# floatingtrees/video-VAE

Hardware: AMD Instinct MI355X
Metric: video frames/sec (fwd+bwd) at Bx3x16x256x256 (higher is better)
Workload: dtype bf16; 1 GPU; C3: full VideoVAE (enc 9 / dec 12 FactoredAttention + 3D-conv UNet) train step, B=4/GPU x 3x16x256x256, bf16 compute, fp32 params, recon+KL loss, clip+Adam; flavour=model, params=170631304, global_batch=4, frames_per_clip=16, parallelism=dp1, launch_mode=hipgraph(fwd+bwd) + eager all-reduce/clip/Adam

## Files before the change

video_vae_amd/csrc/attn_rows.hpp:

```cpp
#pragma once
#include "common.hpp"

namespace {

template <typename T_> struct Vw;
template <> struct Vw<float> { static constexpr int n = 4; };
template <> struct Vw<bf16_t> { static constexpr int n = 8; };

template <typename T_, int D, int LPR> struct Slice {
    static constexpr int DL = D / LPR;
    static constexpr int HL = DL / 2;
    static constexpr int H = D / 2;
    static constexpr int V = Vw<T_>::n < HL ? Vw<T_>::n : HL;
    static_assert(HL % V == 0 && HL >= 4, "slice halves must be whole vectors");
    static __device__ __forceinline__ int ch(int r, int p) { return r < HL ? p * HL + r : H + p * HL + (r - HL); }
    static __device__ __forceinline__ int lo(int p) { return p * HL; }
    static __device__ __forceinline__ int hi(int p) { return H + p * HL; }
};

__device__ __forceinline__ float dpp_xor1(float v) {
    return __int_as_float(__builtin_amdgcn_mov_dpp(__float_as_int(v), 0xB1, 0xf, 0xf, true));
}
__device__ __forceinline__ float dpp_xor2(float v) {
    return __int_as_float(__builtin_amdgcn_mov_dpp(__float_as_int(v), 0x4E, 0xf, 0xf, true));
}
template <int LPR> __device__ __forceinline__ float lpr_sum(float v) {
    static_assert(LPR == 1 || LPR == 2 || LPR == 4, "frames are split over at most a lane quad");
    if (LPR >= 2) v += dpp_xor1(v);
    if (LPR >= 4) v += dpp_xor2(v);
    return v;
}
template <int LPR> __device__ __forceinline__ float frames_sum(float v) { return butterfly_sum<32, LPR>(v); }

template <typename T_, int D, int LPR>
__device__ __forceinline__ void load_row(const T_* __restrict__ row, int p, float (&r)[D / LPR]) {
    using S = Slice<T_, D, LPR>;
#pragma unroll
    for (int half = 0; half < 2; ++half) {
        const T_* src = row + (half ? S::hi(p) : S::lo(p));
#pragma unroll
        for (int c = 0; c < S::HL / S::V; ++c) {
            float t[S::V];
            VecIO<T_, S::V>::load(src + c * S::V, t);
#pragma unroll
            for (int e = 0; e < S::V; ++e) r[half * S::HL + c * S::V + e] = t[e];
        }
    }
}
template <typename T_, int D, int LPR>
__device__ __forceinline__ void store_row(T_* __restrict__ row, int p, const float (&r)[D / LPR]) {
    using S = Slice<T_, D, LPR>;
#pragma unroll
    for (int half = 0; half < 2; ++half) {
        T_* dst = row + (half ? S::hi(p) : S::lo(p));
#pragma unroll
        for (int c = 0; c < S::HL / S::V; ++c) {
            float t[S::V];
#pragma unroll
            for (int e = 0; e < S::V; ++e) t[e] = r[half * S::HL + c * S::V + e];
            VecIO<T_, S::V>::store(dst + c * S::V, t);
        }
    }
}
template <typename T_, int D, int LPR>
__device__ __forceinline__ void load_tab(const float* __restrict__ row, int p, float (&r)[D / LPR]) {
    using S = Slice<T_, D, LPR>;
#pragma unroll
    for (int i = 0; i < S::DL; ++i) r[i] = row[S::ch(i, p)];
}

template <int DL, int LPR, int D>
__device__ __forceinline__ float xhat_row(float (&x)[DL], float eps) {
    float s = 0.f, ss = 0.f;
#pragma unroll
    for (int i = 0; i < DL; ++i) { s += x[i]; ss += x[i] * x[i]; }
    s = lpr_sum<LPR>(s); ss = lpr_sum<LPR>(ss);
    const float mean = s / D;
    float var = ss / D - mean * mean;
    var = var < 0.f ? 0.f : var;
    const float rstd = rsqrtf(var + eps);
#pragma unroll
    for (int i = 0; i < DL; ++i) x[i] = (x[i] - mean) * rstd;
    return rstd;
}

template <typename T_, int D, int LPR>
__device__ __forceinline__ void ln_rope_row(float (&x)[D / LPR], int p, const float* __restrict__ scale, float eps,
                                            const float* __restrict__ cosr, const float* __restrict__ sinr) {
    using S = Slice<T_, D, LPR>;
    xhat_row<S::DL, LPR, D>(x, eps);
#pragma unroll
    for (int i = 0; i < S::HL; ++i) {
        const int cl = S::ch(i, p), chh = S::ch(i + S::HL, p);
        float lo = x[i] * scale[cl], hi = x[i + S::HL] * scale[chh];
        round2<T_>(lo, hi);
        float a = lo * cosr[cl], b = -hi * sinr[cl], c = hi * cosr[chh], e = lo * sinr[chh];
        round2<T_>(a, b);
        round2<T_>(c, e);
        float y0 = a + b, y1 = c + e;
        round2<T_>(y0, y1);
        x[i] = y0; x[i + S::HL] = y1;
    }
}

template <typename T_, int D, int LPR>
__device__ __forceinline__ void rope_ln_bwd_row(float (&g)[D / LPR], float (&xh)[D / LPR], int p, float rstd,
                                                const float* __restrict__ scale, const float* __restrict__ cosr,
                                                const float* __restrict__ sinr) {
    using S = Slice<T_, D, LPR>;
#pragma unroll
    for (int i = 0; i < S::HL; ++i) {
        const float lo = g[i], hi = g[i + S::HL];
        const int cl = S::ch(i, p), chh = S::ch(i + S::HL, p);
        g[i] = lo * cosr[cl] + hi * sinr[chh];
        g[i + S::HL] = hi * cosr[chh] - lo * sinr[cl];
    }
    float sc[S::DL];
    load_tab<T_, D, LPR>(scale, p, sc);
    float s1 = 0.f, s2 = 0.f;
#pragma unroll
    for (int i = 0; i < S::DL; ++i) {
        const float dxh = g[i] * sc[i];
        s1 += dxh; s2 += dxh * xh[i];
    }
    s1 = lpr_sum<LPR>(s1) / D; s2 = lpr_sum<LPR>(s2) / D;
#pragma unroll
    for (int i = 0; i < S::DL; ++i) {
        const float dy = g[i], x = xh[i];
        g[i] = rstd * (dy * sc[i] - s1 - x * s2);
        xh[i] = dy * x;
    }
}

template <typename T_, int D, int LPR>
__device__ __forceinline__ void ln_rope_row_reg(float (&x)[D / LPR], float eps, const float (&sc)[D / LPR], const float (&cs)[D / LPR],
                                                const float (&sn)[D / LPR]) {
    using S = Slice<T_, D, LPR>;
    xhat_row<S::DL, LPR, D>(x, eps);
#pragma unroll
    for (int i = 0; i < S::HL; ++i) {
        float lo = x[i] * sc[i], hi = x[i + S::HL] * sc[i + S::HL];
        round2<T_>(lo, hi);
        float a = lo * cs[i], b = -hi * sn[i], c = hi * cs[i + S::HL], e = lo * sn[i + S::HL];
        round2<T_>(a, b);
        round2<T_>(c, e);
        float y0 = a + b, y1 = c + e;
        round2<T_>(y0, y1);
        x[i] = y0; x[i + S::HL] = y1;
    }
}
template <typename T_, int D, int LPR>
__device__ __forceinline__ void rope_ln_bwd_row_reg(float (&g)[D / LPR], float (&xh)[D / LPR], float rstd, const float (&sc)[D / LPR],
                                                    const float (&cs)[D / LPR], const float (&sn)[D / LPR]) {
    using S = Slice<T_, D, LPR>;
#pragma unroll
    for (int i = 0; i < S::HL; ++i) {
        const float lo = g[i], hi = g[i + S::HL];
        g[i] = lo * cs[i] + hi * sn[i + S::HL];
        g[i + S::HL] = hi * cs[i + S::HL] - lo * sn[i];
    }
    float s1 = 0.f, s2 = 0.f;
#pragma unroll
    for (int i = 0; i < S::DL; ++i) {
        const float dxh = g[i] * sc[i];
        s1 += dxh; s2 += dxh * xh[i];
    }
    s1 = lpr_sum<LPR>(s1) / D; s2 = lpr_sum<LPR>(s2) / D;
#pragma unroll
    for (int i = 0; i < S::DL; ++i) {
        const float dy = g[i], x = xh[i];
        g[i] = rstd * (dy * sc[i] - s1 - x * s2);
        xh[i] = dy * x;
    }
}

}
```

video_vae_amd/csrc/attn_spatial.hip:

```cpp
#include "attn_tile32.hpp"

#ifndef SATTN_PROBE
#define SATTN_PROBE 0
#endif

namespace {

struct SAttnDims { int A, S, H; float eps; };

template <int NT, int S_>
struct RawRows {
    static constexpr int RPP = NT / 4;
    static constexpr int PASSES = (S_ + RPP - 1) / RPP;
    uint4 v[PASSES][2];
    __device__ __forceinline__ void fetch(const bf16_t* __restrict__ src, long tok0, int ld) {
        const int p = threadIdx.x & 3;
#pragma unroll
        for (int i = 0; i < PASSES; ++i) {
            const int row = (threadIdx.x >> 2) + i * RPP;
            if (S_ % RPP == 0 || row < S_) {
                const bf16_t* r = src + (tok0 + row) * ld;
                v[i][0] = *reinterpret_cast<const uint4*>(r + 8 * p);
                v[i][1] = *reinterpret_cast<const uint4*>(r + 32 + 8 * p);
            } else {
                v[i][0] = make_uint4(0u, 0u, 0u, 0u);
                v[i][1] = make_uint4(0u, 0u, 0u, 0u);
            }
        }
    }
    static __device__ __forceinline__ void unpack(const uint4 (&u)[2], float (&x)[16]) {
        const uint32_t w[8] = {u[0].x, u[0].y, u[0].z, u[0].w, u[1].x, u[1].y, u[1].z, u[1].w};
#pragma unroll
        for (int i = 0; i < 8; ++i) { x[2 * i] = __uint_as_float(w[i] << 16); x[2 * i + 1] = __uint_as_float(w[i] & 0xffff0000u); }
    }
    __device__ __forceinline__ void put_raw(unsigned char* img) const {
        const int p = threadIdx.x & 3;
#pragma unroll
        for (int i = 0; i < PASSES; ++i) {
            const int row = (threadIdx.x >> 2) + i * RPP;
            if (S_ % RPP == 0 || row < S_) {
                *reinterpret_cast<uint4*>(img + img_off(row, p)) = v[i][0];
                *reinterpret_cast<uint4*>(img + img_off(row, 4 + p)) = v[i][1];
            }
        }
    }
    template <class Tabs>
    __device__ __forceinline__ void put_norm(unsigned char* img, const float (&sc)[16], float eps, const Tabs& t) const {
        const int p = threadIdx.x & 3;
#pragma unroll
        for (int i = 0; i < PASSES; ++i) {
            const int row = (threadIdx.x >> 2) + i * RPP;
            if (S_ % RPP == 0 || row < S_) {
                float x[16];
                unpack(v[i], x);
                ln_rope_row_reg<bf16_t, SD, 4>(x, eps, sc, t.cs[i], t.sn[i]);
                float lo[8], hi[8];
#pragma unroll
                for (int e = 0; e < 8; ++e) { lo[e] = x[e]; hi[e] = x[8 + e]; }
                VecIO<bf16_t, 8>::store(reinterpret_cast<bf16_t*>(img + img_off(row, p)), lo);
                VecIO<bf16_t, 8>::store(reinterpret_cast<bf16_t*>(img + img_off(row, 4 + p)), hi);
            }
        }
    }
};
template <int NT, int S_>
struct RowTabs {
    static constexpr int RPP = NT / 4, PASSES = (S_ + RPP - 1) / RPP;
    float cs[PASSES][16], sn[PASSES][16];
    __device__ __forceinline__ void fetch(const float* __restrict__ cosT, const float* __restrict__ sinT) {
        const int p = threadIdx.x & 3;
#pragma unroll
        for (int i = 0; i < PASSES; ++i) {
            int row = (threadIdx.x >> 2) + i * RPP;
            if (S_ % RPP != 0 && row >= S_) row = 0;
            load_tab<bf16_t, SD, 4>(cosT + (long)row * SD, p, cs[i]);
            load_tab<bf16_t, SD, 4>(sinT + (long)row * SD, p, sn[i]);
        }
    }
};

template <int NKB>
__global__ __launch_bounds__(256, 2) void sattn_fwd_kernel(const bf16_t* __restrict__ qkv, int ld, bf16_t* __restrict__ out, int ldo,
                                                           float* __restrict__ lse2, const float* __restrict__ q_scale,
                                                           const float* __restrict__ k_scale, const float* __restrict__ cosT,
                                                           const float* __restrict__ sinT, SAttnDims d)
{
    extern __shared__ __attribute__((aligned(16))) unsigned char smem[];
    constexpr int S = 32 * NKB;
    unsigned char* Ks = smem;
    unsigned char* Vs = smem + S * SROW;
    const int lane = threadIdx.x & 63, wave = threadIdx.x >> 6;
    unsigned char* scr = smem + 2 * S * SROW + wave * SCR_BYTES;
    const int a = blockIdx.x / d.H, h = blockIdx.x - a * d.H;
    const int HD = d.H * SD;
    const long tok0 = (long)a * S;
    const bf16_t* base = qkv + h * SD;

    if (!(SATTN_PROBE & 1)) {
        RawRows<256, S> rk, rv;
        RowTabs<256, S> tabs;
        float sck[16];
        rk.fetch(base + HD, tok0, ld);
        tabs.fetch(cosT, sinT);
        load_tab<bf16_t, SD, 4>(k_scale, threadIdx.x & 3, sck);
        rv.fetch(base + 2 * HD, tok0, ld);
        rk.put_norm(Ks, sck, d.eps, tabs);
        rv.put_raw(Vs);
    }
    __syncthreads();

    const int j = lane & 31, kh = lane >> 5;
    const FragAddr fa(lane);
    const float c2 = rsqrtf((float)SD) * 1.44269504088896341f;

    for (int qb = wave; qb < NKB && !(SATTN_PROBE & 2); qb += 4) {
        const int qrow = qb * 32 + j;
        bf16x8 qf[4];
        {
            float x[2][16], cs[2][16], sn[2][16], sc[16];
#pragma unroll
            for (int hf = 0; hf < 2; ++hf) {
                const long rr = qb * 32 + 16 * hf + (lane >> 2);
                load_row<bf16_t, SD, 4>(base + (tok0 + rr) * ld, lane & 3, x[hf]);
                load_tab<bf16_t, SD, 4>(cosT + rr * SD, lane & 3, cs[hf]);
                load_tab<bf16_t, SD, 4>(sinT + rr * SD, lane & 3, sn[hf]);
            }
            load_tab<bf16_t, SD, 4>(q_scale, lane & 3, sc);
#pragma unroll
            for (int hf = 0; hf < 2; ++hf) {
                ln_rope_row_reg<bf16_t, SD, 4>(x[hf], d.eps, sc, cs[hf], sn[hf]);
                wave_lds_fence();
                rows_put(scr, lane, x[hf]);
                wave_lds_fence();
                if ((j >> 4) == hf) {
#pragma unroll
                    for (int ks = 0; ks < 4; ++ks)
                        qf[ks] = *reinterpret_cast<const bf16x8*>(scr + (j & 15) * SROW + (((2 * ks + kh) ^ gsw(j & 15)) << 4));
                }
            }
        }

        constexpr int G = NKB < 4 ? NKB : 4;
        float m = -3.0e38f, l = 0.f;
// ... 2 lines not shown
        for (int dt = 0; dt < 2; ++dt)
#pragma unroll
            for (int e = 0; e < 16; ++e) o[dt][e] = 0.f;
#pragma unroll 1
        for (int kb0 = 0; kb0 < NKB; kb0 += G) {
            f32x16 s[G];
            float mg = m;
#pragma unroll
            for (int g = 0; g < G; ++g) {
                if (kb0 + g < NKB) {
#pragma unroll
                    for (int e = 0; e < 16; ++e) s[g][e] = 0.f;
#pragma unroll
                    for (int ks = 0; ks < 4; ++ks) {
                        s[g] = __builtin_amdgcn_mfma_f32_32x32x16_bf16(fa.rowfrag(Ks, kb0 + g, ks), qf[ks], s[g], 0, 0, 0);
                    }
#pragma unroll
                    for (int e = 0; e < 16; ++e) mg = fmaxf(mg, s[g][e]);
                }
            }
            mg = fmaxf(mg, xor32(mg));
            if (kb0 > 0) {
                const float alpha = exp2_fast((m - mg) * c2);
                l *= alpha;
#pragma unroll
                for (int dt = 0; dt < 2; ++dt)
#pragma unroll
                    for (int e = 0; e < 16; ++e) o[dt][e] *= alpha;
            }
            m = mg;
            const float mc2 = m * c2;
#pragma unroll
            for (int g = 0; g < G; ++g) {
                if (kb0 + g < NKB) {
#pragma unroll
                    for (int u = 0; u < 2; ++u) {
                        float pv[8];
#pragma unroll
                        for (int e = 0; e < 8; ++e) { pv[e] = exp2_fast(__builtin_fmaf(s[g][8 * u + e], c2, -mc2)); l += pv[e]; }
                        const bf16x8 pf = pack8(pv);
#pragma unroll
                        for (int dt = 0; dt < 2; ++dt)
                            o[dt] = __builtin_amdgcn_mfma_f32_32x32x16_bf16(fa.trfrag(Vs, kb0 + g, u, dt), pf, o[dt], 0, 0, 0);
                    }
                }
            }
        }
        l += xor32(l);
        const float inv = 1.f / l;
        float og[2][16];
#pragma unroll
        for (int dt = 0; dt < 2; ++dt)
#pragma unroll
            for (int e = 0; e < 16; ++e) og[dt][e] = o[dt][e] * inv;
#pragma unroll
        for (int hf = 0; hf < 2; ++hf) {
            wave_lds_fence();
            acc_half_put(scr, j, kh, hf, og);
            wave_lds_fence();
            float x[16];
            rows_get(scr, lane, x);
            store_row<bf16_t, SD, 4>(out + (tok0 + qb * 32 + 16 * hf + (lane >> 2)) * ldo + h * SD, lane & 3, x);
        }
        if (kh == 0) lse2[((long)a * d.H + h) * S + qrow] = m * c2 + log2f(l);
    }
}

template <int NKB>
__global__ __launch_bounds__(512) void sattn_bwd_kernel(const bf16_t* __restrict__ qkv, int ld, const bf16_t* __restrict__ out, int ldo,
                                                           const bf16_t* __restrict__ dout, int lddo, const float* __restrict__ lse2,
                                                           bf16_t* __restrict__ dqkv, int lddq, const float* __restrict__ q_scale,
                                                           const float* __restrict__ k_scale, const float* __restrict__ cosT,
                                                           const float* __restrict__ sinT, float* __restrict__ part, SAttnDims d)
{
    extern __shared__ __attribute__((aligned(16))) unsigned char smem[];
    constexpr int S = 32 * NKB;
    unsigned char* Qs = smem;
    unsigned char* Ks = smem + S * SROW;
    unsigned char* Vs = smem + 2 * S * SROW;
    unsigned char* Gs = smem + 3 * S * SROW;
    float* lseS = reinterpret_cast<float*>(smem + 4 * S * SROW);
    float* delS = lseS + S;
    float* red = delS + S;
    const int lane = threadIdx.x & 63, wave = threadIdx.x >> 6;
    unsigned char* scr = reinterpret_cast<unsigned char*>(red + 16 * SD) + wave * SCR_BYTES;
    const int a = blockIdx.x / d.H, h = blockIdx.x - a * d.H;
    const int HD = d.H * SD;
    const long tok0 = (long)a * S;
    const bf16_t* base = qkv + h * SD;
    const bf16_t* gbase = dout + h * SD;
    const int j = lane & 31, kh = lane >> 5;
    const FragAddr fa(lane);
    const float sm_scale = rsqrtf((float)SD);
    const float c2 = sm_scale * 1.44269504088896341f;

    if (!(SATTN_PROBE & 1)) {
        typedef RawRows<512, S> RR;
        RR rv, rg, ro, rq, rk;
        RowTabs<512, S> tabs;
        float scq[16], sck[16];
        rq.fetch(base, tok0, ld);
        rk.fetch(base + HD, tok0, ld);
        tabs.fetch(cosT, sinT);
        load_tab<bf16_t, SD, 4>(q_scale, threadIdx.x & 3, scq);
        load_tab<bf16_t, SD, 4>(k_scale, threadIdx.x & 3, sck);
        rv.fetch(base + 2 * HD, tok0, ld);
        rg.fetch(gbase, tok0, lddo);
        ro.fetch(out + h * SD, tok0, ldo);
        float lse_r[RR::PASSES];
#pragma unroll
        for (int i = 0; i < RR::PASSES; ++i) {
            const int row = (threadIdx.x >> 2) + i * RR::RPP;
            lse_r[i] = row < S ? lse2[((long)a * d.H + h) * S + row] : 0.f;
        }
        rq.put_norm(Qs, scq, d.eps, tabs);
        rk.put_norm(Ks, sck, d.eps, tabs);
        rv.put_raw(Vs);
        rg.put_raw(Gs);
#pragma unroll
        for (int i = 0; i < RR::PASSES; ++i) {
            const int row = (threadIdx.x >> 2) + i * RR::RPP;
            float go[16], oo[16];
            RR::unpack(rg.v[i], go);
            RR::unpack(ro.v[i], oo);
            float dl = 0.f;
#pragma unroll
            for (int e = 0; e < 16; ++e) dl += go[e] * oo[e];
            dl = lpr_sum<4>(dl);
            if ((threadIdx.x & 3) == 0 && row < S) { delS[row] = dl; lseS[row] = lse_r[i]; }
        }
    }
    auto put_v_tile = [&](const float (&g)[2][16], int row0) {
#pragma unroll
        for (int hf = 0; hf < 2; ++hf) {
            wave_lds_fence();
            acc_half_put(scr, j, kh, hf, g);
            wave_lds_fence();
            float x[16];
            rows_get(scr, lane, x);
            store_row<bf16_t, SD, 4>(dqkv + (tok0 + row0 + 16 * hf + (lane >> 2)) * lddq + 2 * HD + h * SD, lane & 3, x);
        }
    };
    struct RowCtx { float xr[2][16], cs[2][16], sn[2][16], sc[16]; };
    auto qk_loads = [&](RowCtx& c, int row0, int which, const float* __restrict__ scale) {
        const int p = lane & 3;
#pragma unroll
        for (int hf = 0; hf < 2; ++hf) {
            const long rr = row0 + 16 * hf + (lane >> 2);
            load_row<bf16_t, SD, 4>(base + which * HD + (tok0 + rr) * ld, p, c.xr[hf]);
            load_tab<bf16_t, SD, 4>(cosT + rr * SD, p, c.cs[hf]);
            load_tab<bf16_t, SD, 4>(sinT + rr * SD, p, c.sn[hf]);
        }
        load_tab<bf16_t, SD, 4>(scale, p, c.sc);
    };
    auto qk_finish = [&](RowCtx& c, const float (&g)[2][16], int row0, int which) {
        const int p = lane & 3;
        float ds[16];
#pragma unroll
        for (int hf = 0; hf < 2; ++hf) {
            const int rr = row0 + 16 * hf + (lane >> 2);
            wave_lds_fence();
            acc_half_put(scr, j, kh, hf, g);
            wave_lds_fence();
            float gx[16];
            rows_get(scr, lane, gx);
            const float rstd = xhat_row<16, 4, SD>(c.xr[hf], d.eps);
            rope_ln_bwd_row_reg<bf16_t, SD, 4>(gx, c.xr[hf], rstd, c.sc, c.cs[hf], c.sn[hf]);
            store_row<bf16_t, SD, 4>(dqkv + (tok0 + rr) * lddq + which * HD + h * SD, p, gx);
#pragma unroll
            for (int i = 0; i < 16; ++i) ds[i] = hf ? ds[i] + c.xr[hf][i] : c.xr[hf][i];
        }
#pragma unroll
        for (int i = 0; i < 16; ++i) {
            const float t = frames_sum<4>(ds[i]);
            if (lane < 4) red[(wave * 2 + which) * SD + Slice<bf16_t, SD, 4>::ch(i, p)] = t;
        }
    };
    static_assert(NKB <= 8, "one key tile and one query tile per wave: the red[] slots are written once");
    for (int i = threadIdx.x; i < 16 * SD; i += 512) red[i] = 0.f;
    __syncthreads();

    for (int kt = wave; kt < NKB && !(SATTN_PROBE & 2); kt += 8) {
        bf16x8 kc[4], vc[4];
#pragma unroll
        for (int ks = 0; ks < 4; ++ks) { kc[ks] = fa.rowfrag(Ks, kt, ks); vc[ks] = fa.rowfrag(Vs, kt, ks); }
        f32x16 dv[2], dk[2];
#pragma unroll
        for (int dt = 0; dt < 2; ++dt)
#pragma unroll
            for (int e = 0; e < 16; ++e) { dv[dt][e] = 0.f; dk[dt][e] = 0.f; }
        bf16x8 qr[4], gr[4];
#pragma unroll
        for (int ks = 0; ks < 4; ++ks) { qr[ks] = fa.rowfrag(Qs, 0, ks); gr[ks] = fa.rowfrag(Gs, 0, ks); }
#pragma unroll 1
        for (int qb = 0; qb < NKB; ++qb) {
            f32x16 s, dp;
#pragma unroll
            for (int e = 0; e < 16; ++e) { s[e] = 0.f; dp[e] = 0.f; }
#pragma unroll
            for (int ks = 0; ks < 4; ++ks) {
                s = __builtin_amdgcn_mfma_f32_32x32x16_bf16(qr[ks], kc[ks], s, 0, 0, 0);
                dp = __builtin_amdgcn_mfma_f32_32x32x16_bf16(gr[ks], vc[ks], dp, 0, 0, 0);
            }
            bf16x8 gt[2][2], qt[2][2];
            float4 l4[4], d4[4];
#pragma unroll
            for (int u = 0; u < 2; ++u)
#pragma unroll
                for (int dt = 0; dt < 2; ++dt) { gt[u][dt] = fa.trfrag(Gs, qb, u, dt); qt[u][dt] = fa.trfrag(Qs, qb, u, dt); }
#pragma unroll
            for (int i = 0; i < 4; ++i) {
                l4[i] = *reinterpret_cast<const float4*>(lseS + qb * 32 + 8 * i + 4 * kh);
                d4[i] = *reinterpret_cast<const float4*>(delS + qb * 32 + 8 * i + 4 * kh);
            }
            {
                const int nb = qb + 1 < NKB ? qb + 1 : qb;
#pragma unroll
                for (int ks = 0; ks < 4; ++ks) { qr[ks] = fa.rowfrag(Qs, nb, ks); gr[ks] = fa.rowfrag(Gs, nb, ks); }
            }
#pragma unroll
            for (int u = 0; u < 2; ++u) {
                float p8[8], s8[8];
#pragma unroll
                for (int hh = 0; hh < 2; ++hh) {
                    const float4 lv = l4[2 * u + hh], dv4 = d4[2 * u + hh];
                    const float lq[4] = {lv.x, lv.y, lv.z, lv.w}, dq4[4] = {dv4.x, dv4.y, dv4.z, dv4.w};
#pragma unroll
                    for (int e = 0; e < 4; ++e) {
                        const float pe = exp2_fast(s[8 * u + 4 * hh + e] * c2 - lq[e]);
                        p8[4 * hh + e] = pe;
                        s8[4 * hh + e] = pe * (dp[8 * u + 4 * hh + e] - dq4[e]);
                    }
                }
                const bf16x8 pf = pack8(p8), sf = pack8(s8);
#pragma unroll
                for (int dt = 0; dt < 2; ++dt) {
                    dv[dt] = __builtin_amdgcn_mfma_f32_32x32x16_bf16(gt[u][dt], pf, dv[dt], 0, 0, 0);
                    dk[dt] = __builtin_amdgcn_mfma_f32_32x32x16_bf16(qt[u][dt], sf, dk[dt], 0, 0, 0);
                }
            }
        }
        RowCtx c;
        qk_loads(c, kt * 32, 1, k_scale);
        float g[2][16];
#pragma unroll
        for (int dt = 0; dt < 2; ++dt)
#pragma unroll
            for (int r = 0; r < 16; ++r) g[dt][r] = dv[dt][r];
        put_v_tile(g, kt * 32);
#pragma unroll
        for (int dt = 0; dt < 2; ++dt)
#pragma unroll
            for (int r = 0; r < 16; ++r) g[dt][r] = dk[dt][r] * sm_scale;
        qk_finish(c, g, kt * 32, 1);
    }

    for (int qt = wave; qt < NKB && !(SATTN_PROBE & 4); qt += 8) {
        const int qrow = qt * 32 + j;
        bf16x8 qc[4], gc[4];
#pragma unroll
        for (int ks = 0; ks < 4; ++ks) { qc[ks] = fa.rowfrag(Qs, qt, ks); gc[ks] = fa.rowfrag(Gs, qt, ks); }
        const float lq = lseS[qrow], dl = delS[qrow];
        f32x16 dq[2];
#pragma unroll
        for (int dt = 0; dt < 2; ++dt)
#pragma unroll
            for (int e = 0; e < 16; ++e) dq[dt][e] = 0.f;
        bf16x8 kr[4], vr[4];
#pragma unroll
        for (int ks = 0; ks < 4; ++ks) { kr[ks] = fa.rowfrag(Ks, 0, ks); vr[ks] = fa.rowfrag(Vs, 0, ks); }
#pragma unroll 1
        for (int kb = 0; kb < NKB; ++kb) {
            f32x16 s, dp;
#pragma unroll
            for (int e = 0; e < 16; ++e) { s[e] = 0.f; dp[e] = 0.f; }
#pragma unroll
            for (int ks = 0; ks < 4; ++ks) {
                s = __builtin_amdgcn_mfma_f32_32x32x16_bf16(kr[ks], qc[ks], s, 0, 0, 0);
                dp = __builtin_amdgcn_mfma_f32_32x32x16_bf16(vr[ks], gc[ks], dp, 0, 0, 0);
            }
            bf16x8 kt2[2][2];
#pragma unroll
            for (int u = 0; u < 2; ++u)
#pragma unroll
                for (int dt = 0; dt < 2; ++dt) kt2[u][dt] = fa.trfrag(Ks, kb, u, dt);
            {
                const int nb = kb + 1 < NKB ? kb + 1 : kb;
#pragma unroll
                for (int ks = 0; ks < 4; ++ks) { kr[ks] = fa.rowfrag(Ks, nb, ks); vr[ks] = fa.rowfrag(Vs, nb, ks); }
            }
#pragma unroll
            for (int u = 0; u < 2; ++u) {
                float s8[8];
#pragma unroll
                for (int e = 0; e < 8; ++e) s8[e] = exp2_fast(s[8 * u + e] * c2 - lq) * (dp[8 * u + e] - dl);
                const bf16x8 sf = pack8(s8);
#pragma unroll
                for (int dt = 0; dt < 2; ++dt)
                    dq[dt] = __builtin_amdgcn_mfma_f32_32x32x16_bf16(kt2[u][dt], sf, dq[dt], 0, 0, 0);
            }
        }
        float g[2][16];
#pragma unroll
        for (int dt = 0; dt < 2; ++dt)
#pragma unroll
            for (int r = 0; r < 16; ++r) g[dt][r] = dq[dt][r] * sm_scale;
        RowCtx c;
        qk_loads(c, qt * 32, 0, q_scale);
        qk_finish(c, g, qt * 32, 0);
    }

    __syncthreads();
    if (threadIdx.x < 2 * SD) {
        const int t = threadIdx.x;
        float tot = 0.f;
#pragma unroll
        for (int w = 0; w < 8; ++w) tot += red[w * 2 * SD + t];
        part[(long)blockIdx.x * 2 * SD + t] = tot;
    }
}

bool sattn_ok(int S, int D, int dtype) { return D == SD && dtype == VVAE_DT_BF16 && S >= 32 && S <= 256 && S % 32 == 0; }

template <int NKB>
int launch_sattn_bwd(const void* qkv, int ld, const void* out, int ldo, const void* dout, int lddo, const float* lse2, void* dqkv, int lddq,
                     const float* qs, const float* ks, const float* cosT, const float* sinT, float* part, SAttnDims d, hipStream_t s)
{
    constexpr int lds = 4 * 32 * NKB * SROW + 2 * 32 * NKB * 4 + 16 * SD * 4 + 8 * SCR_BYTES;
    auto k = sattn_bwd_kernel<NKB>;
    static bool attr_done = false;
    if (!attr_done && lds > 48 * 1024) {
        hipError_t e = hipFuncSetAttribute((const void*)k, hipFuncAttributeMaxDynamicSharedMemorySize, lds);
        if (e != hipSuccess) return (int)e;
        attr_done = true;
    }
    hipLaunchKernelGGL(k, dim3(d.A * d.H), dim3(512), lds, s, (const bf16_t*)qkv, ld, (const bf16_t*)out, ldo, (const bf16_t*)dout, lddo, lse2,
                       (bf16_t*)dqkv, lddq, qs, ks, cosT, sinT, part, d);
    VVAE_LAUNCH_CHECK();
    return 0;
}

template <int NKB>
int launch_sattn_fwd(const void* qkv, int ld, void* out, int ldo, float* lse2, const float* qs, const float* ks, const float* cosT,
                     const float* sinT, SAttnDims d, hipStream_t s)
{
    constexpr int lds = 2 * 32 * NKB * SROW + 4 * SCR_BYTES;
    auto k = sattn_fwd_kernel<NKB>;
    static bool attr_done = false;
    if (!attr_done && lds > 48 * 1024) {
        hipError_t e = hipFuncSetAttribute((const void*)k, hipFuncAttributeMaxDynamicSharedMemorySize, lds);
        if (e != hipSuccess) return (int)e;
        attr_done = true;
    }
    hipLaunchKernelGGL(k, dim3(d.A * d.H), dim3(256), lds, s, (const bf16_t*)qkv, ld, (bf16_t*)out, ldo, lse2, qs, ks, cosT, sinT, d);
    VVAE_LAUNCH_CHECK();
    return 0;
}

}

#define SATTN_DISPATCH(FN, ...)                                                         \
    switch (S / 32) {                                                                   \
        case 1: return FN<1>(__VA_ARGS__); case 2: return FN<2>(__VA_ARGS__);           \
        case 3: return FN<3>(__VA_ARGS__); case 4: return FN<4>(__VA_ARGS__);           \
        case 5: return FN<5>(__VA_ARGS__); case 6: return FN<6>(__VA_ARGS__);           \
        case 7: return FN<7>(__VA_ARGS__); default: return FN<8>(__VA_ARGS__);          \
    }

extern "C" int vvae_spatial_attn_supported(int S, int D, int dtype) { return sattn_ok(S, D, dtype) ? 1 : 0; }

extern "C" int vvae_spatial_attn_fwd(const void* qkv, int ld, void* out, int ldo, float* lse2, const float* q_scale, const float* k_scale,
                                     const float* cos_table, const float* sin_table, int A, int S, int heads, int D, float eps, int dtype,
                                     void* stream)
{
    if (!qkv || !out || !lse2 || !q_scale || !k_scale || !cos_table || !sin_table || A <= 0 || heads <= 0 || !sattn_ok(S, D, dtype) ||
        ld < 3 * heads * D || ldo < heads * D || ld % 8 || ldo % 8 || ((uintptr_t)qkv % 16) || ((uintptr_t)out % 16))
        return VVAE_ERR_BAD_ARG;
    SAttnDims d{A, S, heads, eps};
    hipStream_t s = (hipStream_t)stream;
    SATTN_DISPATCH(launch_sattn_fwd, qkv, ld, out, ldo, lse2, q_scale, k_scale, cos_table, sin_table, d, s);
}

extern "C" int vvae_spatial_attn_bwd(const void* qkv, int ld, const void* out, int ldo, const void* dout, int lddo, const float* lse2,
                                     void* dqkv, int lddq, const float* q_scale, const float* k_scale, const float* cos_table,
                                     const float* sin_table, float* part, int A, int S, int heads, int D, float eps, int dtype, void* stream)
{
    if (!qkv || !out || !dout || !lse2 || !dqkv || !part || !q_scale || !k_scale || !cos_table || !sin_table || A <= 0 || heads <= 0 ||
        !sattn_ok(S, D, dtype) || ld < 3 * heads * D || lddq < 3 * heads * D || ldo < heads * D || lddo < heads * D || ld % 8 || ldo % 8 ||
        lddo % 8 || lddq % 8 || ((uintptr_t)qkv % 16) || ((uintptr_t)out % 16) || ((uintptr_t)dout % 16) || ((uintptr_t)dqkv % 16))
        return VVAE_ERR_BAD_ARG;
    SAttnDims d{A, S, heads, eps};
    hipStream_t s = (hipStream_t)stream;
    SATTN_DISPATCH(launch_sattn_bwd, qkv, ld, out, ldo, dout, lddo, lse2, dqkv, lddq, q_scale, k_scale, cos_table, sin_table, part, d, s);
}
```

video_vae_amd/csrc/attn_temporal_mfma.hip:

```cpp
#include "common.hpp"

namespace tmfma {

typedef __bf16 bf16x8 __attribute__((ext_vector_type(8)));
typedef short s16x4v __attribute__((ext_vector_type(4)));

constexpr int T = 16, D = 64;
constexpr int PITCH = 160;
constexpr int IMG = T * PITCH;

struct Dims { int A, heads, mask_div, inner; float eps; long items; };

__device__ __forceinline__ long token_of(const Dims& d, int a, int row) {
    return (long)(a / d.inner) * T * d.inner + (long)row * d.inner + (a % d.inner);
}

__device__ __forceinline__ void unpack8(const uint4& r, float* v) {
    const uint32_t w[4] = {r.x, r.y, r.z, r.w};
#pragma unroll
    for (int i = 0; i < 4; ++i) { v[2 * i] = __uint_as_float(w[i] << 16); v[2 * i + 1] = __uint_as_float(w[i] & 0xffff0000u); }
}
__device__ __forceinline__ uint4 pack8(const float* v) {
    uint32_t w[4];
#pragma unroll
    for (int i = 0; i < 4; ++i) w[i] = (uint32_t)f2bf(v[2 * i]) | ((uint32_t)f2bf(v[2 * i + 1]) << 16);
    return make_uint4(w[0], w[1], w[2], w[3]);
}
__device__ __forceinline__ bf16x8 frag8(const uint4& r) { return __builtin_bit_cast(bf16x8, r); }
__device__ __forceinline__ s16x4v pack4(float a, float b, float c, float e) {
    s16x4v r = {(short)f2bf(a), (short)f2bf(b), (short)f2bf(c), (short)f2bf(e)};
    return r;
}
__device__ __forceinline__ s16x4v tr4(const unsigned char* p) {
    typedef __attribute__((address_space(3))) s16x4v* lds_ptr;
    return __builtin_amdgcn_ds_read_tr16_b64_v4i16((lds_ptr)p);
}
__device__ __forceinline__ f32x4 mfma32(const bf16x8& a, const bf16x8& b, f32x4 c) { return __builtin_amdgcn_mfma_f32_16x16x32_bf16(a, b, c, 0, 0, 0); }
__device__ __forceinline__ f32x4 mfma16(const s16x4v& a, const s16x4v& b, f32x4 c) { return __builtin_amdgcn_mfma_f32_16x16x16bf16_1k(a, b, c, 0, 0, 0); }

__device__ __forceinline__ float psum(float v) { return butterfly_sum<32, 16>(v); }
__device__ __forceinline__ float pmax(float v) { v = fmaxf(v, xor_lane<32>(v)); return fmaxf(v, xor_lane<16>(v)); }

__device__ __forceinline__ float xhat16(float (&x)[16], float eps) {
    float s = 0.f, ss = 0.f;
#pragma unroll
    for (int i = 0; i < 16; ++i) { s += x[i]; ss += x[i] * x[i]; }
    s = psum(s); ss = psum(ss);
    const float mean = s * (1.f / D);
    float var = ss * (1.f / D) - mean * mean;
    var = var < 0.f ? 0.f : var;
    const float rstd = rsqrtf(var + eps);
#pragma unroll
    for (int i = 0; i < 16; ++i) x[i] = (x[i] - mean) * rstd;
    return rstd;
}
__device__ __forceinline__ void ln_rope16(float (&x)[16], const float* __restrict__ sc, float eps, const float* __restrict__ cs,
                                          const float* __restrict__ sn) {
    xhat16(x, eps);
#pragma unroll
    for (int i = 0; i < 8; ++i) {
        float lo = x[i] * sc[i], hi = x[i + 8] * sc[i + 8];
        round2<bf16_t>(lo, hi);
        float a = lo * cs[i], b = -hi * sn[i], c = hi * cs[i + 8], e = lo * sn[i + 8];
        round2<bf16_t>(a, b);
        round2<bf16_t>(c, e);
        float y0 = a + b, y1 = c + e;
        round2<bf16_t>(y0, y1);
        x[i] = y0; x[i + 8] = y1;
    }
}
__device__ __forceinline__ void tab16(const float* __restrict__ row, int p, float (&r)[16]) {
    const float4* lo = reinterpret_cast<const float4*>(row + 8 * p);
    const float4* hi = reinterpret_cast<const float4*>(row + 32 + 8 * p);
    const float4 a = lo[0], b = lo[1], c = hi[0], e = hi[1];
    r[0] = a.x; r[1] = a.y; r[2] = a.z; r[3] = a.w; r[4] = b.x; r[5] = b.y; r[6] = b.z; r[7] = b.w;
    r[8] = c.x; r[9] = c.y; r[10] = c.z; r[11] = c.w; r[12] = e.x; r[13] = e.y; r[14] = e.z; r[15] = e.w;
}
__device__ __forceinline__ void norm_row(const bf16_t* __restrict__ g, int p, const float (&sc)[16], float eps, const float (&cs)[16],
                                         const float (&sn)[16], uint4& f0, uint4& f1) {
    float x[16];
    unpack8(*reinterpret_cast<const uint4*>(g + 8 * p), x);
    unpack8(*reinterpret_cast<const uint4*>(g + 32 + 8 * p), x + 8);
    ln_rope16(x, sc, eps, cs, sn);
    f0 = pack8(x); f1 = pack8(x + 8);
}
__device__ __forceinline__ void put_row(unsigned char* img, int t, int p, const uint4& f0, const uint4& f1) {
    *reinterpret_cast<uint4*>(img + t * PITCH + 16 * p) = f0;
    *reinterpret_cast<uint4*>(img + t * PITCH + 64 + 16 * p) = f1;
}
__device__ __forceinline__ void wave_lds_fence() {
    __builtin_amdgcn_wave_barrier();
    __builtin_amdgcn_s_waitcnt(0xc07f);
    __builtin_amdgcn_wave_barrier();
}
__device__ __forceinline__ s16x4v tr_rows(const unsigned char* img, int p, int i, int tile) {
    return tr4(img + (4 * p + (i >> 2)) * PITCH + 32 * tile + 8 * (i & 3));
}

__global__ __launch_bounds__(256) void tattn16_fwd_mfma(const bf16_t* __restrict__ qkv, int ld, bf16_t* __restrict__ out, int ldo,
                                                       float* __restrict__ lse, const float* __restrict__ q_scale,
                                                       const float* __restrict__ k_scale, const float* __restrict__ cosT,
                                                       const float* __restrict__ sinT, const uint8_t* __restrict__ mask, Dims d)
{
    __shared__ __attribute__((aligned(16))) unsigned char smem[4 * IMG];
    const int lane = threadIdx.x & 63, wave = threadIdx.x >> 6;
    const int t = lane & 15, p = lane >> 4;
    const long item = (long)blockIdx.x * 4 + wave;
    if (item >= d.items) return;
    const int a = (int)(item / d.heads), h = (int)(item % d.heads);
    const int HD = d.heads * D;
    const long tok = token_of(d, a, t);
    const bf16_t* g = qkv + tok * ld + h * D;
    unsigned char* vimg = smem + wave * IMG;

// ... 317 lines not shown
```

video_vae_amd/csrc/attn_tile32.hpp:

```cpp
#pragma once
#include "attn_rows.hpp"

namespace {

typedef __bf16 bf16x8 __attribute__((ext_vector_type(8)));
typedef short s16x4v __attribute__((ext_vector_type(4)));

constexpr int SD = 64;
constexpr int SROW = SD * 2;

__device__ __forceinline__ int gsw(int row) { return (((row >> 1) & 1) << 2) | (((row >> 3) & 1) << 1) | ((row >> 2) & 1); }

__device__ __forceinline__ float xor32(float v) { return xor_lane<32>(v); }

__device__ __forceinline__ bf16x8 pack8(const float (&v)[8])
{
    s16x8 r;
#pragma unroll
    for (int e = 0; e < 8; ++e) r[e] = (short)f2bf(v[e]);
    return __builtin_bit_cast(bf16x8, r);
}

__device__ __forceinline__ bf16x8 tr_pair(const unsigned char* p0, const unsigned char* p1)
{
    typedef __attribute__((address_space(3))) s16x4v* lds_ptr;
    const s16x4v lo = __builtin_amdgcn_ds_read_tr16_b64_v4i16((lds_ptr)p0);
    const s16x4v hi = __builtin_amdgcn_ds_read_tr16_b64_v4i16((lds_ptr)p1);
    s16x8 v = {lo[0], lo[1], lo[2], lo[3], hi[0], hi[1], hi[2], hi[3]};
    return __builtin_bit_cast(bf16x8, v);
}

__device__ __forceinline__ int img_off(int row, int c) { return row * SROW + ((c ^ gsw(row)) << 4); }
struct FragAddr {
    int row[4], tr[2][2];
    __device__ __forceinline__ FragAddr(int lane) {
        const int j = lane & 31, kh = lane >> 5, p4 = lane & 3, qr = (lane >> 2) & 3, mh = (lane >> 4) & 1;
        const int gj = gsw(j), gl = (((qr >> 1) & 1) << 2) | kh;
#pragma unroll
        for (int ks = 0; ks < 4; ++ks) row[ks] = j * SROW + (((2 * ks + kh) ^ gj) << 4);
#pragma unroll
        for (int dt = 0; dt < 2; ++dt)
#pragma unroll
            for (int x = 0; x < 2; ++x)
                tr[dt][x] = (4 * kh + qr + 8 * x) * SROW + (((2 * (2 * dt + mh) + (p4 >> 1)) ^ (gl | (x << 1))) << 4) + (p4 & 1) * 8;
    }
    __device__ __forceinline__ bf16x8 rowfrag(const unsigned char* img, int blk, int ks) const {
        return *reinterpret_cast<const bf16x8*>(img + blk * 32 * SROW + row[ks]);
    }
    __device__ __forceinline__ bf16x8 trfrag(const unsigned char* img, int blk, int u, int dt) const {
        const unsigned char* b = img + (blk * 32 + 16 * u) * SROW;
        return tr_pair(b + tr[dt][0], b + tr[dt][1]);
    }
};

constexpr int SCR_BYTES = 16 * SROW;

__device__ __forceinline__ void wave_lds_fence()
{
    __builtin_amdgcn_wave_barrier();
    __builtin_amdgcn_s_waitcnt(0xc07f);
    __builtin_amdgcn_wave_barrier();
}

__device__ __forceinline__ void acc_half_put(unsigned char* scr, int j, int kh, int hf, const float (&g)[2][16])
{
    if ((j >> 4) == hf) {
        const int row = j & 15, gs = gsw(row);
        unsigned char* r = scr + row * SROW + kh * 8;
#pragma unroll
        for (int dt = 0; dt < 2; ++dt)
#pragma unroll
            for (int rg = 0; rg < 4; ++rg) {
                uint2 o;
                o.x = (uint32_t)f2bf(g[dt][4 * rg]) | ((uint32_t)f2bf(g[dt][4 * rg + 1]) << 16);
                o.y = (uint32_t)f2bf(g[dt][4 * rg + 2]) | ((uint32_t)f2bf(g[dt][4 * rg + 3]) << 16);
                *reinterpret_cast<uint2*>(r + (((4 * dt + rg) ^ gs) << 4)) = o;
            }
    }
}
__device__ __forceinline__ void rows_put(unsigned char* scr, int lane, const float (&x)[16])
{
    const int row = lane >> 2, p = lane & 3;
    float lo[8], hi[8];
#pragma unroll
    for (int e = 0; e < 8; ++e) { lo[e] = x[e]; hi[e] = x[8 + e]; }
    VecIO<bf16_t, 8>::store(reinterpret_cast<bf16_t*>(scr + img_off(row, p)), lo);
    VecIO<bf16_t, 8>::store(reinterpret_cast<bf16_t*>(scr + img_off(row, 4 + p)), hi);
}
__device__ __forceinline__ void rows_get(const unsigned char* scr, int lane, float (&x)[16])
{
    const int row = lane >> 2, p = lane & 3;
    float lo[8], hi[8];
    VecIO<bf16_t, 8>::load(reinterpret_cast<const bf16_t*>(scr + img_off(row, p)), lo);
    VecIO<bf16_t, 8>::load(reinterpret_cast<const bf16_t*>(scr + img_off(row, 4 + p)), hi);
#pragma unroll
    for (int e = 0; e < 8; ++e) { x[e] = lo[e]; x[8 + e] = hi[e]; }
}

__device__ __forceinline__ float exp2_fast(float x) { return __builtin_amdgcn_exp2f(x); }

}
```

video_vae_amd/csrc/common.hpp:

```cpp
#pragma once
#include <hip/hip_runtime.h>
#include <stdint.h>

#define VVAE_DT_F32 0
#define VVAE_DT_BF16 1

#define VVAE_ERR_BAD_ARG 1001
#define VVAE_ERR_WORKSPACE 1002
#define VVAE_ERR_LIBRARY 1003

typedef uint16_t bf16_t;

typedef float f32x4 __attribute__((ext_vector_type(4)));
typedef float f32x16 __attribute__((ext_vector_type(16)));
typedef short s16x8 __attribute__((ext_vector_type(8)));
typedef short s16x4 __attribute__((ext_vector_type(4)));

__device__ __forceinline__ float bf2f(bf16_t b) { return __uint_as_float(((uint32_t)b) << 16); }

__device__ __forceinline__ bf16_t f2bf(float f) {
    __bf16 h = (__bf16)f;
    return __builtin_bit_cast(bf16_t, h);
}

__device__ __forceinline__ float ldf(const float* p) { return *p; }
__device__ __forceinline__ float ldf(const bf16_t* p) { return bf2f(*p); }
__device__ __forceinline__ void stf(float* p, float v) { *p = v; }
__device__ __forceinline__ void stf(bf16_t* p, float v) { *p = f2bf(v); }

template <typename T> __device__ __forceinline__ float round_to(float v);
template <> __device__ __forceinline__ float round_to<float>(float v) { return v; }
template <> __device__ __forceinline__ float round_to<bf16_t>(float v) { return bf2f(f2bf(v)); }
template <typename T> __device__ __forceinline__ void round2(float& a, float& b);
template <> __device__ __forceinline__ void round2<float>(float&, float&) {}
template <> __device__ __forceinline__ void round2<bf16_t>(float& a, float& b) {
    typedef __bf16 bf16x2_t __attribute__((ext_vector_type(2)));
    typedef float f32x2_t __attribute__((ext_vector_type(2)));
    const f32x2_t v = {a, b};
    const uint32_t w = __builtin_bit_cast(uint32_t, __builtin_convertvector(v, bf16x2_t));
    a = __uint_as_float(w << 16);
    b = __uint_as_float(w & 0xffff0000u);
}

__device__ __forceinline__ void vvae_phase_barrier()
{
    __builtin_amdgcn_sched_barrier(0);
    __builtin_amdgcn_s_barrier();
    __builtin_amdgcn_sched_barrier(0);
}

template <typename T, int VEC> struct VecIO;

template <> struct VecIO<float, 4> {
    static __device__ __forceinline__ void load(const float* p, float (&v)[4]) {
        float4 t = *reinterpret_cast<const float4*>(p);
        v[0] = t.x; v[1] = t.y; v[2] = t.z; v[3] = t.w;
    }
    static __device__ __forceinline__ void store(float* p, const float (&v)[4]) {
        *reinterpret_cast<float4*>(p) = make_float4(v[0], v[1], v[2], v[3]);
    }
};
template <> struct VecIO<float, 1> {
    static __device__ __forceinline__ void load(const float* p, float (&v)[1]) { v[0] = *p; }
    static __device__ __forceinline__ void store(float* p, const float (&v)[1]) { *p = v[0]; }
};
template <> struct VecIO<bf16_t, 8> {
    static __device__ __forceinline__ void load(const bf16_t* p, float (&v)[8]) {
        uint4 t = *reinterpret_cast<const uint4*>(p);
        uint32_t w[4] = {t.x, t.y, t.z, t.w};
#pragma unroll
        for (int i = 0; i < 4; ++i) {
            v[2 * i] = __uint_as_float(w[i] << 16);
            v[2 * i + 1] = __uint_as_float(w[i] & 0xffff0000u);
        }
    }
    static __device__ __forceinline__ void store(bf16_t* p, const float (&v)[8]) {
        uint32_t w[4];
#pragma unroll
        for (int i = 0; i < 4; ++i) w[i] = (uint32_t)f2bf(v[2 * i]) | ((uint32_t)f2bf(v[2 * i + 1]) << 16);
        *reinterpret_cast<uint4*>(p) = make_uint4(w[0], w[1], w[2], w[3]);
    }
};
template <> struct VecIO<bf16_t, 4> {
    static __device__ __forceinline__ void load(const bf16_t* p, float (&v)[4]) {
        uint2 t = *reinterpret_cast<const uint2*>(p);
        v[0] = __uint_as_float(t.x << 16); v[1] = __uint_as_float(t.x & 0xffff0000u);
        v[2] = __uint_as_float(t.y << 16); v[3] = __uint_as_float(t.y & 0xffff0000u);
    }
    static __device__ __forceinline__ void store(bf16_t* p, const float (&v)[4]) {
        uint2 t;
        t.x = (uint32_t)f2bf(v[0]) | ((uint32_t)f2bf(v[1]) << 16);
        t.y = (uint32_t)f2bf(v[2]) | ((uint32_t)f2bf(v[3]) << 16);
        *reinterpret_cast<uint2*>(p) = t;
    }
};
template <> struct VecIO<bf16_t, 1> {
    static __device__ __forceinline__ void load(const bf16_t* p, float (&v)[1]) { v[0] = bf2f(*p); }
    static __device__ __forceinline__ void store(bf16_t* p, const float (&v)[1]) { *p = f2bf(v[0]); }
};

template <typename T> struct VecWidth;
template <> struct VecWidth<float> { static constexpr int value = 4; };
template <> struct VecWidth<bf16_t> { static constexpr int value = 8; };

template <int CTRL> __device__ __forceinline__ unsigned dpp_u32(unsigned v) {
    return (unsigned)__builtin_amdgcn_update_dpp(0, (int)v, CTRL, 0xf, 0xf, true);
}
template <int O> __device__ __forceinline__ unsigned xor_lane_u32(unsigned v) {
    static_assert(O == 1 || O == 2 || O == 4 || O == 8 || O == 16 || O == 32, "one address bit at a time");
    if constexpr (O == 1) return dpp_u32<0xB1>(v);
    else if constexpr (O == 2) return dpp_u32<0x4E>(v);
    else if constexpr (O == 4) return dpp_u32<0x1B>(dpp_u32<0x141>(v));
    else if constexpr (O == 8) return dpp_u32<0x128>(v);
    else if constexpr (O == 16) {
        const auto r = __builtin_amdgcn_permlane16_swap(v, v, false, false);
        return (threadIdx.x & 16) ? r[0] : r[1];
    } else {
        const auto r = __builtin_amdgcn_permlane32_swap(v, v, false, false);
        return (threadIdx.x & 32) ? r[0] : r[1];
    }
}
template <int O> __device__ __forceinline__ float xor_lane(float v) { return __uint_as_float(xor_lane_u32<O>(__float_as_uint(v))); }
template <int O> __device__ __forceinline__ double xor_lane(double v) {
    const unsigned long long u = __builtin_bit_cast(unsigned long long, v);
    const unsigned lo = xor_lane_u32<O>((unsigned)u), hi = xor_lane_u32<O>((unsigned)(u >> 32));
    return __builtin_bit_cast(double, ((unsigned long long)hi << 32) | lo);
}
template <int HI, int LO, typename F> __device__ __forceinline__ F butterfly_sum(F v) {
    static_assert(HI >= LO && LO >= 1, "bit range");
    v += xor_lane<HI>(v);
    if constexpr (HI > LO) return butterfly_sum<HI / 2, LO>(v);
    else return v;
}

__device__ __forceinline__ float wave_sum(float v) { return butterfly_sum<32, 1>(v); }
__device__ __forceinline__ double wave_sum(double v) { return butterfly_sum<32, 1>(v); }

__device__ __forceinline__ float sigmoidf_(float x) { return __builtin_amdgcn_rcpf(1.0f + __expf(-x)); }

static inline int ceil_div(long a, long b) { return (int)((a + b - 1) / b); }

__global__ static void vvae_zero_words_kernel(uint32_t* __restrict__ p, long n)
{
    for (long i = (long)blockIdx.x * blockDim.x + threadIdx.x; i < n; i += (long)gridDim.x * blockDim.x) p[i] = 0u;
}
static inline hipError_t vvae_zero_async(void* p, size_t bytes, hipStream_t s)
{
    const long n = (long)(bytes / 4);
    if (n <= 0) return hipSuccess;
    long blocks = (n + 255) / 256;
    if (blocks > 1024) blocks = 1024;
    hipLaunchKernelGGL(vvae_zero_words_kernel, dim3((unsigned)blocks), dim3(256), 0, s, (uint32_t*)p, n);
    return hipGetLastError();
}
__global__ static void vvae_reduce_rows_kernel(const float* __restrict__ part, int rows, long stride, int ncols, float* __restrict__ out0, int n0,
                                               float* __restrict__ out1)
{
    __shared__ float red[8][32];
    const int cl = threadIdx.x & 31, rl = threadIdx.x >> 5;
    const int c = blockIdx.x * 32 + cl;
    float s = 0.f;
    if (c < ncols) {
        for (int r0 = rl; r0 < rows; r0 += 8 * 8) {
            float v[8];
#pragma unroll
            for (int i = 0; i < 8; ++i) {
                const int r = r0 + 8 * i;
                v[i] = r < rows ? part[(long)r * stride + c] : 0.f;
            }
#pragma unroll
            for (int i = 0; i < 8; ++i) s += v[i];
        }
    }
    red[rl][cl] = s;
    __syncthreads();
    if (rl == 0 && c < ncols) {
        const float t = ((red[0][cl] + red[1][cl]) + (red[2][cl] + red[3][cl])) + ((red[4][cl] + red[5][cl]) + (red[6][cl] + red[7][cl]));
        if (c < n0) out0[c] = t;
        else if (out1) out1[c - n0] = t;
    }
}

#define VVAE_LAUNCH_CHECK() do { hipError_t e_ = hipGetLastError(); if (e_ != hipSuccess) return (int)e_; } while (0)
```

Before: 1913 frames/s.

## Cache LayerNorm row stats in LDS for spatial attention backward and pack bf16 pairwise

The spatial attention backward kernel now writes each Q/K row's mean and rstd to LDS during the forward-normalise pass and reuses them in the gradient pass, instead of recomputing the row reduction with lane shuffles. Scalar bf16 conversions are replaced with a paired float-to-bf16x2 vector conversion in several pack helpers. Butterfly sums for offsets 16/32 now add both outputs of permlane swap directly, avoiding a lane-dependent select. The kernel uses more LDS, which may reduce occupancy.

```diff
diff --git a/video_vae_amd/csrc/attn_rows.hpp b/video_vae_amd/csrc/attn_rows.hpp
--- a/video_vae_amd/csrc/attn_rows.hpp
+++ b/video_vae_amd/csrc/attn_rows.hpp
@@ -47,6 +47,13 @@
         }
     }
 }
+template <typename T_, int V> struct RowIO : VecIO<T_, V> {};
+template <> struct RowIO<bf16_t, 8> : VecIO<bf16_t, 8> {
+    static __device__ __forceinline__ void store(bf16_t* p, const float (&v)[8]) {
+        *reinterpret_cast<uint4*>(p) = make_uint4(pack2bf(v[0], v[1]), pack2bf(v[2], v[3]), pack2bf(v[4], v[5]), pack2bf(v[6], v[7]));
+    }
+};
+
 template <typename T_, int D, int LPR>
 __device__ __forceinline__ void store_row(T_* __restrict__ row, int p, const float (&r)[D / LPR]) {
     using S = Slice<T_, D, LPR>;
@@ -58,7 +65,7 @@
             float t[S::V];
 #pragma unroll
             for (int e = 0; e < S::V; ++e) t[e] = r[half * S::HL + c * S::V + e];
-            VecIO<T_, S::V>::store(dst + c * S::V, t);
+            RowIO<T_, S::V>::store(dst + c * S::V, t);
         }
     }
 }
@@ -70,17 +77,26 @@
 }
 
 template <int DL, int LPR, int D>
-__device__ __forceinline__ float xhat_row(float (&x)[DL], float eps) {
+__device__ __forceinline__ void row_stats(const float (&x)[DL], float eps, float& mean, float& rstd) {
     float s = 0.f, ss = 0.f;
 #pragma unroll
     for (int i = 0; i < DL; ++i) { s += x[i]; ss += x[i] * x[i]; }
     s = lpr_sum<LPR>(s); ss = lpr_sum<LPR>(ss);
-    const float mean = s / D;
+    mean = s / D;
     float var = ss / D - mean * mean;
     var = var < 0.f ? 0.f : var;
-    const float rstd = rsqrtf(var + eps);
+    rstd = rsqrtf(var + eps);
+}
+template <int DL>
+__device__ __forceinline__ void xhat_apply(float (&x)[DL], float mean, float rstd) {
 #pragma unroll
     for (int i = 0; i < DL; ++i) x[i] = (x[i] - mean) * rstd;
+}
+template <int DL, int LPR, int D>
+__device__ __forceinline__ float xhat_row(float (&x)[DL], float eps) {
+    float mean, rstd;
+    row_stats<DL, LPR, D>(x, eps, mean, rstd);
+    xhat_apply<DL>(x, mean, rstd);
     return rstd;
 }
 
@@ -133,10 +149,9 @@
 }
 
 template <typename T_, int D, int LPR>
-__device__ __forceinline__ void ln_rope_row_reg(float (&x)[D / LPR], float eps, const float (&sc)[D / LPR], const float (&cs)[D / LPR],
-                                                const float (&sn)[D / LPR]) {
+__device__ __forceinline__ void scale_rope_row_reg(float (&x)[D / LPR], const float (&sc)[D / LPR], const float (&cs)[D / LPR],
+                                                   const float (&sn)[D / LPR]) {
     using S = Slice<T_, D, LPR>;
-    xhat_row<S::DL, LPR, D>(x, eps);
 #pragma unroll
     for (int i = 0; i < S::HL; ++i) {
         float lo = x[i] * sc[i], hi = x[i + S::HL] * sc[i + S::HL];
@@ -148,6 +163,12 @@
         round2<T_>(y0, y1);
         x[i] = y0; x[i + S::HL] = y1;
     }
+}
+template <typename T_, int D, int LPR>
+__device__ __forceinline__ void ln_rope_row_reg(float (&x)[D / LPR], float eps, const float (&sc)[D / LPR], const float (&cs)[D / LPR],
+                                                const float (&sn)[D / LPR]) {
+    xhat_row<D / LPR, LPR, D>(x, eps);
+    scale_rope_row_reg<T_, D, LPR>(x, sc, cs, sn);
 }
 template <typename T_, int D, int LPR>
 __device__ __forceinline__ void rope_ln_bwd_row_reg(float (&g)[D / LPR], float (&xh)[D / LPR], float rstd, const float (&sc)[D / LPR],
diff --git a/video_vae_amd/csrc/attn_spatial.hip b/video_vae_amd/csrc/attn_spatial.hip
--- a/video_vae_amd/csrc/attn_spatial.hip
+++ b/video_vae_amd/csrc/attn_spatial.hip
@@ -45,7 +45,8 @@
         }
     }
     template <class Tabs>
-    __device__ __forceinline__ void put_norm(unsigned char* img, const float (&sc)[16], float eps, const Tabs& t) const {
+    __device__ __forceinline__ void put_norm(unsigned char* img, const float (&sc)[16], float eps, const Tabs& t,
+                                             float2* stats = nullptr) const {
         const int p = threadIdx.x & 3;
 #pragma unroll
         for (int i = 0; i < PASSES; ++i) {
@@ -53,12 +54,16 @@
             if (S_ % RPP == 0 || row < S_) {
                 float x[16];
                 unpack(v[i], x);
-                ln_rope_row_reg<bf16_t, SD, 4>(x, eps, sc, t.cs[i], t.sn[i]);
+                float mean, rstd;
+                row_stats<16, 4, SD>(x, eps, mean, rstd);
+                if (stats && p == 0) stats[row] = make_float2(mean, rstd);
+                xhat_apply<16>(x, mean, rstd);
+                scale_rope_row_reg<bf16_t, SD, 4>(x, sc, t.cs[i], t.sn[i]);
                 float lo[8], hi[8];
 #pragma unroll
                 for (int e = 0; e < 8; ++e) { lo[e] = x[e]; hi[e] = x[8 + e]; }
-                VecIO<bf16_t, 8>::store(reinterpret_cast<bf16_t*>(img + img_off(row, p)), lo);
-                VecIO<bf16_t, 8>::store(reinterpret_cast<bf16_t*>(img + img_off(row, 4 + p)), hi);
+                RowIO<bf16_t, 8>::store(reinterpret_cast<bf16_t*>(img + img_off(row, p)), lo);
+                RowIO<bf16_t, 8>::store(reinterpret_cast<bf16_t*>(img + img_off(row, 4 + p)), hi);
             }
         }
     }
@@ -227,8 +232,10 @@
     float* lseS = reinterpret_cast<float*>(smem + 4 * S * SROW);
     float* delS = lseS + S;
     float* red = delS + S;
+    float2* qstat = reinterpret_cast<float2*>(red + 16 * SD);
+    float2* kstat = qstat + S;
     const int lane = threadIdx.x & 63, wave = threadIdx.x >> 6;
-    unsigned char* scr = reinterpret_cast<unsigned char*>(red + 16 * SD) + wave * SCR_BYTES;
+    unsigned char* scr = reinterpret_cast<unsigned char*>(kstat + S) + wave * SCR_BYTES;
     const int a = blockIdx.x / d.H, h = blockIdx.x - a * d.H;
     const int HD = d.H * SD;
     const long tok0 = (long)a * S;
@@ -258,8 +265,8 @@
             const int row = (threadIdx.x >> 2) + i * RR::RPP;
             lse_r[i] = row < S ? lse2[((long)a * d.H + h) * S + row] : 0.f;
         }
-        rq.put_norm(Qs, scq, d.eps, tabs);
-        rk.put_norm(Ks, sck, d.eps, tabs);
+        rq.put_norm(Qs, scq, d.eps, tabs, qstat);
+        rk.put_norm(Ks, sck, d.eps, tabs, kstat);
         rv.put_raw(Vs);
         rg.put_raw(Gs);
 #pragma unroll
@@ -309,8 +316,9 @@
             wave_lds_fence();
             float gx[16];
             rows_get(scr, lane, gx);
-            const float rstd = xhat_row<16, 4, SD>(c.xr[hf], d.eps);
-            rope_ln_bwd_row_reg<bf16_t, SD, 4>(gx, c.xr[hf], rstd, c.sc, c.cs[hf], c.sn[hf]);
+            const float2 st = (which ? kstat : qstat)[rr];
+            xhat_apply<16>(c.xr[hf], st.x, st.y);
+            rope_ln_bwd_row_reg<bf16_t, SD, 4>(gx, c.xr[hf], st.y, c.sc, c.cs[hf], c.sn[hf]);
             store_row<bf16_t, SD, 4>(dqkv + (tok0 + rr) * lddq + which * HD + h * SD, p, gx);
 #pragma unroll
             for (int i = 0; i < 16; ++i) ds[i] = hf ? ds[i] + c.xr[hf][i] : c.xr[hf][i];
@@ -471,7 +479,8 @@
 int launch_sattn_bwd(const void* qkv, int ld, const void* out, int ldo, const void* dout, int lddo, const float* lse2, void* dqkv, int lddq,
                      const float* qs, const float* ks, const float* cosT, const float* sinT, float* part, SAttnDims d, hipStream_t s)
 {
-    constexpr int lds = 4 * 32 * NKB * SROW + 2 * 32 * NKB * 4 + 16 * SD * 4 + 8 * SCR_BYTES;
+    constexpr int lds = 4 * 32 * NKB * SROW + 2 * 32 * NKB * 4 + 16 * SD * 4 + 2 * 32 * NKB * 8 + 8 * SCR_BYTES;
+    static_assert(lds <= 160 * 1024, "LDS of one CU");
     auto k = sattn_bwd_kernel<NKB>;
     static bool attr_done = false;
     if (!attr_done && lds > 48 * 1024) {
diff --git a/video_vae_amd/csrc/attn_temporal_mfma.hip b/video_vae_amd/csrc/attn_temporal_mfma.hip
--- a/video_vae_amd/csrc/attn_temporal_mfma.hip
+++ b/video_vae_amd/csrc/attn_temporal_mfma.hip
@@ -23,13 +23,12 @@
 __device__ __forceinline__ uint4 pack8(const float* v) {
     uint32_t w[4];
 #pragma unroll
-    for (int i = 0; i < 4; ++i) w[i] = (uint32_t)f2bf(v[2 * i]) | ((uint32_t)f2bf(v[2 * i + 1]) << 16);
+    for (int i = 0; i < 4; ++i) w[i] = pack2bf(v[2 * i], v[2 * i + 1]);
     return make_uint4(w[0], w[1], w[2], w[3]);
 }
 __device__ __forceinline__ bf16x8 frag8(const uint4& r) { return __builtin_bit_cast(bf16x8, r); }
 __device__ __forceinline__ s16x4v pack4(float a, float b, float c, float e) {
-    s16x4v r = {(short)f2bf(a), (short)f2bf(b), (short)f2bf(c), (short)f2bf(e)};
-    return r;
+    return __builtin_bit_cast(s16x4v, make_uint2(pack2bf(a, b), pack2bf(c, e)));
 }
 __device__ __forceinline__ s16x4v tr4(const unsigned char* p) {
     typedef __attribute__((address_space(3))) s16x4v* lds_ptr;
diff --git a/video_vae_amd/csrc/attn_tile32.hpp b/video_vae_amd/csrc/attn_tile32.hpp
--- a/video_vae_amd/csrc/attn_tile32.hpp
+++ b/video_vae_amd/csrc/attn_tile32.hpp
@@ -15,9 +15,7 @@
 
 __device__ __forceinline__ bf16x8 pack8(const float (&v)[8])
 {
-    s16x8 r;
-#pragma unroll
-    for (int e = 0; e < 8; ++e) r[e] = (short)f2bf(v[e]);
+    const uint4 r = make_uint4(pack2bf(v[0], v[1]), pack2bf(v[2], v[3]), pack2bf(v[4], v[5]), pack2bf(v[6], v[7]));
     return __builtin_bit_cast(bf16x8, r);
 }
 
@@ -72,8 +70,8 @@
 #pragma unroll
             for (int rg = 0; rg < 4; ++rg) {
                 uint2 o;
-                o.x = (uint32_t)f2bf(g[dt][4 * rg]) | ((uint32_t)f2bf(g[dt][4 * rg + 1]) << 16);
-                o.y = (uint32_t)f2bf(g[dt][4 * rg + 2]) | ((uint32_t)f2bf(g[dt][4 * rg + 3]) << 16);
+                o.x = pack2bf(g[dt][4 * rg], g[dt][4 * rg + 1]);
+                o.y = pack2bf(g[dt][4 * rg + 2], g[dt][4 * rg + 3]);
                 *reinterpret_cast<uint2*>(r + (((4 * dt + rg) ^ gs) << 4)) = o;
             }
     }
@@ -84,8 +82,8 @@
     float lo[8], hi[8];
 #pragma unroll
     for (int e = 0; e < 8; ++e) { lo[e] = x[e]; hi[e] = x[8 + e]; }
-    VecIO<bf16_t, 8>::store(reinterpret_cast<bf16_t*>(scr + img_off(row, p)), lo);
-    VecIO<bf16_t, 8>::store(reinterpret_cast<bf16_t*>(scr + img_off(row, 4 + p)), hi);
+    RowIO<bf16_t, 8>::store(reinterpret_cast<bf16_t*>(scr + img_off(row, p)), lo);
+    RowIO<bf16_t, 8>::store(reinterpret_cast<bf16_t*>(scr + img_off(row, 4 + p)), hi);
 }
 __device__ __forceinline__ void rows_get(const unsigned char* scr, int lane, float (&x)[16])
 {
diff --git a/video_vae_amd/csrc/common.hpp b/video_vae_amd/csrc/common.hpp
--- a/video_vae_amd/csrc/common.hpp
+++ b/video_vae_amd/csrc/common.hpp
@@ -31,13 +31,16 @@
 template <typename T> __device__ __forceinline__ float round_to(float v);
 template <> __device__ __forceinline__ float round_to<float>(float v) { return v; }
 template <> __device__ __forceinline__ float round_to<bf16_t>(float v) { return bf2f(f2bf(v)); }
+__device__ __forceinline__ uint32_t pack2bf(float a, float b) {
+    typedef __bf16 bf16x2_t __attribute__((ext_vector_type(2)));
+    typedef float f32x2_t __attribute__((ext_vector_type(2)));
+    const f32x2_t v = {a, b};
+    return __builtin_bit_cast(uint32_t, __builtin_convertvector(v, bf16x2_t));
+}
 template <typename T> __device__ __forceinline__ void round2(float& a, float& b);
 template <> __device__ __forceinline__ void round2<float>(float&, float&) {}
 template <> __device__ __forceinline__ void round2<bf16_t>(float& a, float& b) {
-    typedef __bf16 bf16x2_t __attribute__((ext_vector_type(2)));
-    typedef float f32x2_t __attribute__((ext_vector_type(2)));
-    const f32x2_t v = {a, b};
-    const uint32_t w = __builtin_bit_cast(uint32_t, __builtin_convertvector(v, bf16x2_t));
+    const uint32_t w = pack2bf(a, b);
     a = __uint_as_float(w << 16);
     b = __uint_as_float(w & 0xffff0000u);
 }
@@ -126,9 +129,21 @@
     const unsigned lo = xor_lane_u32<O>((unsigned)u), hi = xor_lane_u32<O>((unsigned)(u >> 32));
     return __builtin_bit_cast(double, ((unsigned long long)hi << 32) | lo);
 }
+template <int O> __device__ __forceinline__ float add_xor_lane(float v) {
+    if constexpr (O == 16) {
+        const auto r = __builtin_amdgcn_permlane16_swap(__float_as_uint(v), __float_as_uint(v), false, false);
+        return __uint_as_float(r[0]) + __uint_as_float(r[1]);
+    } else if constexpr (O == 32) {
+        const auto r = __builtin_amdgcn_permlane32_swap(__float_as_uint(v), __float_as_uint(v), false, false);
+        return __uint_as_float(r[0]) + __uint_as_float(r[1]);
+    } else {
+        return v + xor_lane<O>(v);
+    }
+}
+template <int O> __device__ __forceinline__ double add_xor_lane(double v) { return v + xor_lane<O>(v); }
 template <int HI, int LO, typename F> __device__ __forceinline__ F butterfly_sum(F v) {
     static_assert(HI >= LO && LO >= 1, "bit range");
-    v += xor_lane<HI>(v);
+    v = add_xor_lane<HI>(v);
     if constexpr (HI > LO) return butterfly_sum<HI / 2, LO>(v);
     else return v;
 }
```

Measured after the change: 1923 frames/s (median of 6 runs). About the same (+0.5%).
